# ejcanalesr/multicomponent-T2-toolbox

Hardware: AMD Instinct MI355X
Metric: voxels/sec (whole node) at nTE=32, nT2=60; max |MWF-ref| (higher is better)
Workload: dtype f64

## Files before the change

### multicomponent-t2-toolbox_amd/csrc/fit_kernel.hpp

```cpp
#pragma once
#include <hip/hip_runtime.h>
#include <math.h>
#include <stdint.h>

#include "../../include/met2_hip.h"
#include "abi_common.hpp"
#include "nnls_wave.hpp"
#include "objectives.hpp"

using namespace met2;

struct SortBufs {
    int *key;
    int *perm;
    int *hist;
    int *cursor;
    int *bucket_start;
    int *chunk_start;
    int *queue;
    int *xq;
    int *err;
    int *ovf;
};

#ifndef MET2_BAYES_TABLE
#define MET2_BAYES_TABLE 10
#endif
#define MET2_GCV_LR 6
constexpr int LC_SAVE_DOUBLES = 18;

struct FitArgs {
    int n, m, nfa, kmax, waves, chunk;
    int wave_doubles;
    int method, nlam, maxfun;
    double x2_factor, t2sparc_lambda, xtol;
    double cut_m, cut_ie;
    double lam_lo, lam_hi;
    int all_queued;
    double log_detL;
    const double *Dfa;
    const double *Bfa;
    const double *Dtfa;
    const double *Aq;
    const double *kband;
    const double *lband;
    const double *Kd;
    const double *lam_grid;
    const double *t2s;
    const double *data;
    int64_t vs, es;
    SortBufs sb;
    double *fsol, *sig, *reg, *lam, *maps;
    int32_t *status;
    int64_t nvox;
    const char *seed;
    const double *btab;
    int nbtab, btab_stride;
    double *chol;
    int chol_stride;
    double *big;
    int big_stride;
    double *lc_save;
    int *lc_at;
    int lc_cap;
    double blam[MET2_BAYES_TABLE];
    int test_switches = 0;
    static constexpr int TEST_REFAC_PAIR = 1;
    static constexpr int TEST_SUBST_REF = 2;
    unsigned long long *refac_count = nullptr;
};

#ifndef MET2_UNI_MASK
#define MET2_UNI_MASK 37
#endif
constexpr bool uni_brent(int method, int nb)
{
    const int base = method >= 10 ? method - 10 : method;
    const int bit = base == MET2_X2 ? 0 : ((base == MET2_GCV || base == MET2_GCV_LR) ? 2 : (base == MET2_BAYESREG ? 4 : -1));
    return bit >= 0 && ((MET2_UNI_MASK >> (bit + (nb == 2 ? 1 : 0))) & 1);
}
template <bool PIN>
__device__ __forceinline__ double uni(double v)
{
    if constexpr (PIN) {
    const unsigned long long u = (unsigned long long)__double_as_longlong(v);
    const unsigned lo = (unsigned)__builtin_amdgcn_readfirstlane((int)(unsigned)u), hi = (unsigned)__builtin_amdgcn_readfirstlane((int)(unsigned)(u >> 32));
    return __longlong_as_double((long long)(((unsigned long long)hi << 32) | lo));
    } else return v;
}
#define MET2_UNI_PIN() do { a = uni<PIN>(a); b = uni<PIN>(b); fulc = uni<PIN>(fulc); nfc = uni<PIN>(nfc); xf = uni<PIN>(xf); rat = uni<PIN>(rat); e = uni<PIN>(e); \
                            x = uni<PIN>(x); fx = uni<PIN>(fx); ffulc = uni<PIN>(ffulc); fnfc = uni<PIN>(fnfc); } while (0)

template <bool PIN, class F, class G>
__device__ __forceinline__ double fminbound_dev(F &&fn, G &&on_best, double x1, double x2, double xatol, int maxfun, int &flag)
{
    const double sqrt_eps = sqrt(2.2e-16);
    const double golden_mean = 0.5 * (3.0 - sqrt(5.0));
    double a = x1, b = x2;
    double fulc = a + golden_mean * (b - a);
    double nfc = fulc, xf = fulc;
    double rat = 0.0, e = 0.0;
    double x = xf;
    double fx = fn(x);
    on_best();
    int num = 1;
    flag = 0;
    double fu = INFINITY;
    double ffulc = fx, fnfc = fx;
    double xm = 0.5 * (a + b);
    double tol1 = sqrt_eps * fabs(xf) + xatol / 3.0;
    double tol2 = 2.0 * tol1;
    while (fabs(xf - xm) > (tol2 - 0.5 * (b - a))) {
        bool golden = true;
        if (fabs(e) > tol1) {
            golden = false;
            double r = (xf - nfc) * (fx - ffulc);
            double q = (xf - fulc) * (fx - fnfc);
            double p = (xf - fulc) * q - (xf - nfc) * r;
            q = 2.0 * (q - r);
            if (q > 0.0) p = -p;
            q = fabs(q);
            r = e;
            e = rat;
            if ((fabs(p) < fabs(0.5 * q * r)) && (p > q * (a - xf)) && (p < q * (b - xf))) {
                rat = (p + 0.0) / q;
                x = xf + rat;
                if (((x - a) < tol2) || ((b - x) < tol2)) {
                    double d = xm - xf;
                    double si = (double)((d > 0.0) - (d < 0.0) + (d == 0.0));
                    rat = tol1 * si;
                }
            } else golden = true;
        }
        if (golden) {
            e = (xf >= xm) ? a - xf : b - xf;
            rat = golden_mean * e;
        }
        double si = (double)((rat > 0.0) - (rat < 0.0) + (rat == 0.0));
        double ar = fabs(rat);
        x = xf + si * (ar > tol1 ? ar : tol1);
        MET2_UNI_PIN();
        fu = fn(x);
        num++;
        if (fu <= fx) {
            if (x >= xf) a = xf; else b = xf;
            fulc = nfc; ffulc = fnfc;
            nfc = xf; fnfc = fx;
            xf = x; fx = fu;
            on_best();
        } else {
            if (x < xf) a = x; else b = x;
// ... 547 lines not shown
                    const double ld0 = rec[A.btab_stride - 1];
                    if (fabs(ld0) <= 1.79769313486231570815e308) { tab.U0 = rec; tab.logdet0 = ld0; }
                }
            }
            ++ev;
            return bayes_objective<NB>(S, bd, st, bc, x, b, lane, tab, cholG);
        }, []() {}, BIG ? A.lam_lo : 1e-8, BIG ? A.lam_hi : 2.0, A.xtol, A.maxfun, flag);
        if (flag == 1) stat |= MET2_ST_BRENT_MAXFUN;
        if (bc.failed) stat |= MET2_ST_CHOLFAIL;
        if (!(NB == 2 && (st.itmax_hit & 2))) solve_warm<NB, ONE, BIG>(S, bd, st, lam, true, lane);
        regv = lamv = lam;
    } else if (METHOD == MET2_GCV || METHOD == MET2_GCV_LR) {
        int flag, overflow = 0;
        GcvCache<NB> gc; gc.valid = 0; gc.next = 0;
        if (have_seed) seed_load<NB>(st, A.seed, seed_k, fa, lane);
        double lam = fminbound_dev<uni_brent(METHOD, NB)>([&](double x) {
            if (NB == 2 && (st.itmax_hit & 2)) return 0.0;
            solve_warm<NB, ONE, BIG>(S, bd, st, x, true, lane);
            return gcv_objective<NB, METHOD == MET2_GCV_LR>(S, bd, st, x, b, lane, overflow, gc);
        }, []() {}, BIG ? A.lam_lo : 1e-8, BIG ? A.lam_hi : 10.0, A.xtol, A.maxfun, flag);
        if (flag == 1) stat |= MET2_ST_BRENT_MAXFUN;
        if (overflow) stat |= MET2_ST_KOVERFLOW;
        if (!(NB == 2 && (st.itmax_hit & 2))) solve_warm<NB, ONE, BIG>(S, bd, st, lam, true, lane);
        regv = lamv = lam;
    }
    if (METHOD >= 10) {
        constexpr int BASE = METHOD - 10;
        double SSE = 1.0; BayesCtx bc; bc.failed = 0; bc.log_detL = A.log_detL; bc.beta = 1.0;
        if (BASE == MET2_X2 || BASE == MET2_BAYESREG) {
            nnls_solve<NB>(S, bd, st, 0.0, false, lane);
            SSE = sse_of<NB>(S, st, b, lane);
            int nnz = 0;
#pragma unroll
            for (int bb = 0; bb < NB; ++bb) nnz += __popcll(ballot((lane + 64 * bb < n) && (st.x[bb] > 0.0)));
            double dof = (double)(m - nnz); dof = dof < 1.0 ? 1.0 : dof;
            const double sigma = sqrt(SSE / dof);
            bc.beta = 1.0 / (sigma * sigma);
        }
        double keep = 0.0; int overflow = 0;
        GcvCache<NB> gc; gc.valid = 0; gc.next = 0;
        for (int i = 0; i < A.nlam; ++i) {
            const double x = A.lam_grid[i];
            nnls_solve<NB>(S, bd, st, x, true, lane);
            double val;
            if (BASE == MET2_X2) val = fabs(sse_of<NB>(S, st, b, lane) - A.x2_factor * SSE) / SSE;
            else if (BASE == MET2_GCV || BASE == MET2_GCV_LR) val = gcv_objective<NB, BASE == MET2_GCV_LR>(S, bd, st, x, b, lane, overflow, gc);
            else val = bayes_objective<NB>(S, bd, st, bc, x, b, lane);
            if (lane == i) keep = val;
        }
        if (lane < n) A.fsol[(size_t)v * n + lane] = keep;
        if (NB == 2 && lane + 64 < n) A.fsol[(size_t)v * n + lane + 64] = 0.0;
        if (lane == 0) { A.reg[v] = 0.0; if (A.status) A.status[v] = stat | (overflow ? MET2_ST_KOVERFLOW : 0); }
        return false;
    }
    if (st.itmax_hit & 1) stat |= MET2_ST_ITMAX;
    if (st.itmax_hit & 2) stat |= MET2_ST_KOVERFLOW;
    MET2_CYC_END(0, c_vox);
    MET2_CYC_FLUSH(st);

    double xs[NB];
#pragma unroll
    for (int bb = 0; bb < NB; ++bb) {
        xs[bb] = st.x[bb] * km;
        if (lane + 64 * bb < n) A.fsol[(size_t)v * n + lane + 64 * bb] = xs[bb]; else xs[bb] = 0.0;
    }
    if (A.sig) {
        double sg = model_signal<NB>(S, st, lane) * km;
        if (lane < m) A.sig[(size_t)v * m + lane] = sg;
    }
    if (A.maps) write_metrics<NB>(ml, xs, true, A.maps, A.nvox, v, lane);
    if (lane == 0) {
        A.reg[v] = regv;
        if (A.lam) A.lam[v] = lamv;
        if (A.status) A.status[v] = stat;
    }
    return !BIG && !queued && (st.itmax_hit & 2) != 0;
}

__device__ __forceinline__ void fit_shared(const FitArgs &A, WaveShared &S, double *sR, int wslot)
{
    S.R = sR; S.n = A.n; S.m = A.m; S.kmax = A.kmax; S.rcap = A.wave_doubles; S.K = A.Kd; S.kband = A.kband; S.Dt = nullptr; S.DtG = A.Dtfa; S.dtstride = A.m; S.buffer_rows = true; S.reorder = true; S.have_bdiag = false; S.bdiag[0] = S.bdiag[1] = 0.0;
    S.B = A.Bfa; S.D = A.Dfa; S.bstride = A.n; S.dstride = A.n;
    S.Rg = A.big ? A.big + (size_t)wslot * (size_t)A.big_stride : nullptr; S.gbase = col_base(A.kmax);
    S.refac_pair = (A.test_switches & FitArgs::TEST_REFAC_PAIR) != 0; S.subst_ref = (A.test_switches & FitArgs::TEST_SUBST_REF) != 0; S.refac_count = A.refac_count;
}
template <int METHOD>
__device__ __forceinline__ void fit_shared_fa(const FitArgs &A, WaveShared &S, int fa)
{
    const int n = A.n, m = A.m;
    S.B = A.Bfa + (size_t)fa * n * n; S.D = A.Dfa + (size_t)fa * m * n; S.Dt = A.Dtfa + (size_t)fa * m * n;
    S.DtG = ((METHOD >= 10 ? METHOD - 10 : METHOD) == MET2_GCV_LR) ? A.Aq + (size_t)fa * n * MET2_GCV_LR_RANK : S.Dt;
}

template <int METHOD, int NB>
__device__ __attribute__((noinline)) void fit_voxel_spill(const FitArgs *Ap, big_lds_dp sRl, int64_t v, int fa, int wslot, int qslot, int seed_cap)
{
    const int lane = big_lane();
    double *sR = (double *)sRl;
    FitArgs A;
    {
        static_assert(sizeof(FitArgs) % 4 == 0, "FitArgs is copied word by word");
        const int *src = (const int *)Ap;
        int *dst = (int *)&A;
#pragma unroll
        for (int i = 0; i < (int)(sizeof(FitArgs) / 4); ++i) dst[i] = big_rfl(src[i]);
    }
    v = (int64_t)big_rfl((u64)v); fa = big_rfl(fa); wslot = big_rfl(wslot); qslot = big_rfl(qslot); seed_cap = big_rfl(seed_cap);
    WaveShared S;
    fit_shared(A, S, sR, wslot);
    fit_shared_fa<METHOD>(A, S, fa);
    Band<NB> bd;
    load_band<NB>(bd, A.kband, A.lband, lane);
    MetricLanes<NB> ml;
    metric_lanes<NB>(ml, A.t2s, A.n, A.cut_m, A.cut_ie, lane);
    const int seed_k = (MET2_SEED && A.seed) ? ((const SeedRec *)A.seed)[fa].k : 0;
    const bool have_seed = seed_k > 0 && seed_k <= seed_cap;
    (void)fit_voxel<METHOD, NB, true>(A, S, bd, ml, v, fa, seed_k, have_seed, lane, wslot, qslot);
}

template <int METHOD, int NB, bool SECOND>
__global__ __launch_bounds__(64 * method_max_waves(METHOD, NB)) void fit_kernel(FitArgs A)
{
    extern __shared__ __attribute__((aligned(16))) double smem[];
    const int lane = lane_id(), wave = (int)(threadIdx.x >> 6);
    const int n = A.n, m = A.m, kmax = A.kmax;
    const int tri = A.wave_doubles;
    double *sR = smem + (size_t)wave * tri;

    const int wslot = (int)(blockIdx.x * (unsigned)A.waves + (unsigned)wave);
    WaveShared S;
    fit_shared(A, S, sR, wslot);
    Band<NB> bd;
    load_band<NB>(bd, A.kband, A.lband, lane);
    MetricLanes<NB> ml;
    metric_lanes<NB>(ml, A.t2s, n, A.cut_m, A.cut_ie, lane);

    if constexpr (!SECOND) {
    const int nchunks = A.sb.chunk_start[A.nfa];
    for (int round = 0; round <= nchunks; ++round) {
        int c = nchunks;
        if (lane == 0) {
            const int xcd = (int)(blockIdx.x & 7u);
            for (int t = 0; t < 8; ++t) {
                const int q = (xcd + t) & 7;
                const int qlo = (int)(((int64_t)nchunks * q) >> 3), qhi = (int)(((int64_t)nchunks * (q + 1)) >> 3);
                if (qlo >= qhi) continue;
                const int i = atomicAdd(A.sb.xq + q, 1);
                if (i < qhi - qlo) { c = qlo + i; break; }
            }
        }
        c = __builtin_amdgcn_readfirstlane(c);
        MET2_STAT(5, round);
        if (c >= nchunks) break;
        int lo = 0, hi = A.nfa;
        while (hi - lo > 1) { int mid = (lo + hi) >> 1; if (A.sb.chunk_start[mid] <= c) lo = mid; else hi = mid; }
        const int fa = lo;
        const int first = A.sb.bucket_start[fa] + (c - A.sb.chunk_start[fa]) * A.chunk;
        const int cnt = min(A.chunk, A.sb.bucket_start[fa + 1] - first);
        fit_shared_fa<METHOD>(A, S, fa);
        const int seed_k = (MET2_SEED && A.seed) ? ((const SeedRec *)A.seed)[fa].k : 0;
        const bool have_seed = seed_k > 0 && seed_k <= kmax;
        for (int slot = 0; slot < cnt; ++slot) {
            MET2_STAT(4, slot);
            const int64_t v = A.sb.perm[first + slot];

            if (fit_voxel<METHOD, NB, false>(A, S, bd, ml, v, fa, seed_k, have_seed, lane, wslot, -1) && A.big) {
                if (lane == 0) A.sb.ovf[atomicAdd(A.sb.err + 1, 1)] = (int)v;
// ... 44 lines not shown
```

### multicomponent-t2-toolbox_amd/csrc/met2_fit_nnls_lcurve.hip

```cpp
#ifdef MET2_SPLIT_TU
#define MET2_REFAC_PACKED 1
#include "fit_kernel.hpp"
template int launch_fit_nb<0, 1, false>(const FitArgs &, const LaunchGeom &, hipStream_t);
template int launch_fit_nb<0, 2, false>(const FitArgs &, const LaunchGeom &, hipStream_t);
template int launch_fit_nb<1, 1, false>(const FitArgs &, const LaunchGeom &, hipStream_t);
template int launch_fit_nb<1, 2, false>(const FitArgs &, const LaunchGeom &, hipStream_t);
template int launch_fit_nb<3, 1, false>(const FitArgs &, const LaunchGeom &, hipStream_t);
template int launch_fit_nb<3, 2, false>(const FitArgs &, const LaunchGeom &, hipStream_t);
template int launch_fit_nb<0, 1, true>(const FitArgs &, const LaunchGeom &, hipStream_t);
template int launch_fit_nb<0, 2, true>(const FitArgs &, const LaunchGeom &, hipStream_t);
template int launch_fit_nb<1, 1, true>(const FitArgs &, const LaunchGeom &, hipStream_t);
template int launch_fit_nb<1, 2, true>(const FitArgs &, const LaunchGeom &, hipStream_t);
template int launch_fit_nb<3, 1, true>(const FitArgs &, const LaunchGeom &, hipStream_t);
template int launch_fit_nb<3, 2, true>(const FitArgs &, const LaunchGeom &, hipStream_t);
#endif
```

### multicomponent-t2-toolbox_amd/csrc/met2_fit_x2_nb1.hip

```cpp
#ifdef MET2_SPLIT_TU
#define MET2_REFAC_PACKED 1
#include "fit_kernel.hpp"
template int launch_fit_nb<2, 1, false>(const FitArgs &, const LaunchGeom &, hipStream_t);
template int launch_fit_nb<12, 1, false>(const FitArgs &, const LaunchGeom &, hipStream_t);
#endif
```

### multicomponent-t2-toolbox_amd/csrc/met2_hip.hip

```cpp
#include <hip/hip_runtime.h>
#include <math.h>
#include <stddef.h>
#include <stdint.h>
#include <stdio.h>
#include <stdlib.h>
#include <string.h>
#include <string>
#include <vector>

#include "../../include/met2_hip.h"
#include "abi_common.hpp"
#include "nnls_wave.hpp"
#include "objectives.hpp"
#include "fit_kernel.hpp"

using namespace met2;

#ifdef MET2_SPLIT_TU
extern template int launch_fit_nb<0, 1, false>(const FitArgs &, const LaunchGeom &, hipStream_t);
extern template int launch_fit_nb<0, 2, false>(const FitArgs &, const LaunchGeom &, hipStream_t);
extern template int launch_fit_nb<1, 1, false>(const FitArgs &, const LaunchGeom &, hipStream_t);
extern template int launch_fit_nb<1, 2, false>(const FitArgs &, const LaunchGeom &, hipStream_t);
extern template int launch_fit_nb<2, 1, false>(const FitArgs &, const LaunchGeom &, hipStream_t);
extern template int launch_fit_nb<2, 2, false>(const FitArgs &, const LaunchGeom &, hipStream_t);
// ... 1632 lines not shown
      fprintf(stderr, "[met2] spill-over voxels: solver calls=%llu, with spill-over legs=%llu | cycles plain=%llu spill=%llu (refactor in slot %llu) | appends=%llu removals=%llu refactors=%llu | k start sum=%llu end sum=%llu\n",
              bs[0], bs[1], bs[2], bs[3], bs[9], bs[4], bs[5], bs[6], bs[8], bs[7]); }
#endif
#ifdef MET2_LOOPSTATS
    int ls[8];
    HIPCHK(hipMemcpyFromSymbol(ls, HIP_SYMBOL(met2::g_loopstats), sizeof(ls)));
    fprintf(stderr, "[met2] loop maxima: tries=%d sweeps=%d outer=%d iter=%d taken=%d round=%d jacobi_sweeps=%d last_sweep_rotations=%d\n", ls[0], ls[1], ls[2], ls[3], ls[4], ls[5], ls[6], ls[7]);
#endif
    fflush(stderr);
    return MET2_OK;
}

static int fit_impl(met2_plan *p, int32_t method, int64_t nvox, const double *data, int64_t voxel_stride, int64_t echo_stride,
                    const double *fa_index, const uint8_t *mask, double *fsol, double *sig, double *reg, double *lam, double *maps,
                    int32_t *status, void *stream, bool sync)
{
    if (!p) return fail(MET2_E_INVALID, "NULL plan");
    if (voxel_stride == 0 || echo_stride == 0) return fail(MET2_E_INVALID, "zero stride");
    if (nvox == 0) return MET2_OK;
    if (!data || !fsol || !reg) return fail(MET2_E_INVALID, "NULL argument");
    if (nvox < 0 || nvox > 0x7fffffff) return fail(MET2_E_INVALID, "nvox out of range");
    if (!p->have_dict) return fail(MET2_E_STATE, "no dictionary in the plan");
    if (method != MET2_NNLS && !p->have_pen) return fail(MET2_E_STATE, "no penalty matrix set");
    if (maps && !p->have_t2) return fail(MET2_E_STATE, "metrics requested but no T2 grid set");
    const bool objgrid = method >= 10;
    if (objgrid) { method -= 10; if (method != MET2_X2 && method != MET2_GCV && method != MET2_BAYESREG) return fail(MET2_E_INVALID, "no objective for this method"); }
    if (method < 0 || method > MET2_BAYESREG) return fail(MET2_E_INVALID, "unknown method");
    if (objgrid && p->nlam > p->n_t2) return fail(MET2_E_UNSUPPORTED, "objective grid longer than n_t2");
    USE_DEVICE(p->opt.device);
    hipStream_t s = (hipStream_t)stream;
    if (p->err_pending && p->err_stream != s)
        return fail(MET2_E_STATE, "fits are pending on another stream of this plan: call met2_plan_finish on it first (one plan serves one stream at a time)");
    int rc = ensure_sort_bufs(p, nvox);
    if (rc) return rc;
    const int kmeth = kernel_method(p, method);
    const int kfast = objgrid ? 0 : fast_kmax(p, kmeth);
    LaunchGeom g;
    rc = fit_geometry(p, objgrid ? kmeth + 10 : kmeth, g, kfast, 0, nvox);
    if (rc) return rc;
    if (!p->have_pen) {
        HIPCHK(hipMemsetAsync(p->dKband, 0, sizeof(double) * 5 * 128, s));
        HIPCHK(hipMemsetAsync(p->dLband, 0, sizeof(double) * 5 * 128, s));
        HIPCHK(hipMemsetAsync(p->dKd, 0, sizeof(double) * (size_t)p->n_t2 * p->n_t2, s));
    }
    if (!p->have_t2) HIPCHK(hipMemsetAsync(p->dT2, 0, sizeof(double) * 128, s));
    SortBufs sb = sort_bufs(p);
    hipLaunchKernelGGL(reset_sort_kernel, dim3(1), dim3(256), 0, s, sb, p->n_fa, p->err_pending ? 1 : 0);
    const int nbs = (int)((nvox + MET2_SORT_BLOCK - 1) / MET2_SORT_BLOCK);
    const size_t sort_lds = sizeof(int) * 2 * ((size_t)p->n_fa + 1);
    if (sort_lds > 48 * 1024) {
        if (sort_lds > 150 * 1024) return fail(MET2_E_UNSUPPORTED, "more than 19 000 flip angles (or ROIs) in one plan");
        HIPCHK(hipFuncSetAttribute((const void *)classify_kernel, hipFuncAttributeMaxDynamicSharedMemorySize, (int)sort_lds));
        HIPCHK(hipFuncSetAttribute((const void *)scatter_kernel, hipFuncAttributeMaxDynamicSharedMemorySize, (int)sort_lds));
        HIPCHK(hipFuncSetAttribute((const void *)scan_kernel, hipFuncAttributeMaxDynamicSharedMemorySize, (int)sort_lds));
    }
    int chunk = (method <= MET2_T2SPARC) ? 8 : 1;
    chunk = tuning_env("MET2_CHUNK", 1, 1024, chunk);
    const bool dbg = test_switch("MET2_DEBUG");
    if (dbg) { HIPCHK(hipStreamSynchronize(s)); fprintf(stderr, "[met2] fit: nvox=%lld grid=%d block=%d lds=%d\n", (long long)nvox, g.grid, g.block, g.lds); fflush(stderr); }
    hipLaunchKernelGGL(classify_kernel, dim3(nbs), dim3(MET2_SORT_BLOCK), sort_lds, s, nvox, p->n_te, p->n_fa, data, voxel_stride, echo_stride, fa_index, mask, 1, sb, status);
    hipLaunchKernelGGL(scan_kernel, dim3(1), dim3(256), sort_lds, s, p->n_fa, chunk, sb);
    if (dbg) { HIPCHK(hipStreamSynchronize(s)); fprintf(stderr, "[met2] classify done\n"); fflush(stderr); }
    hipLaunchKernelGGL(scatter_kernel, dim3(nbs), dim3(MET2_SORT_BLOCK), sort_lds, s, nvox, p->n_fa, sb);
    HIPCHK(hipGetLastError());
    if (dbg) {
        HIPCHK(hipStreamSynchronize(s));
        std::vector<int> hs(4 * (size_t)(p->n_fa + 1) + 8);
        HIPCHK(hipMemcpy(hs.data(), p->dSmall, sizeof(int) * hs.size(), hipMemcpyDeviceToHost));
        fprintf(stderr, "[met2] sort done: fitted=%d chunks=%d\n", hs[2 * (p->n_fa + 1) + p->n_fa], hs[3 * (p->n_fa + 1) + p->n_fa]); fflush(stderr);
    }

    FitArgs A;
    A.n = p->n_t2; A.m = p->n_te; A.nfa = p->n_fa; A.kmax = g.kmax; A.waves = g.waves; A.chunk = chunk; A.wave_doubles = g.wave_doubles;
    A.method = method; A.nlam = p->nlam;
    A.maxfun = p->opt.brent_maxfun > 0 ? p->opt.brent_maxfun : (method == MET2_BAYESREG ? 200 : 300);
    A.x2_factor = p->opt.x2_factor; A.t2sparc_lambda = p->opt.t2sparc_lambda; A.xtol = p->opt.brent_xtol;
    A.cut_m = p->opt.t2_myelin_cut; A.cut_ie = p->opt.t2_ie_cut;
    A.lam_lo = method == MET2_GCV ? p->opt.gcv_lo : (method == MET2_BAYESREG ? p->opt.bayes_lo : p->opt.x2_lo);
    A.lam_hi = method == MET2_GCV ? p->opt.gcv_hi : (method == MET2_BAYESREG ? p->opt.bayes_hi : p->opt.x2_hi);
    A.log_detL = p->log_detL;
    A.Dfa = p->dD; A.Bfa = p->dB; A.Dtfa = p->dDt; A.Aq = p->dAq; A.kband = p->dKband; A.lband = p->dLband; A.Kd = p->dKd; A.lam_grid = p->dLam; A.t2s = p->dT2;
    A.data = data; A.vs = voxel_stride; A.es = echo_stride; A.sb = sb; A.fsol = fsol; A.sig = sig; A.reg = reg; A.lam = lam; A.maps = maps; A.status = status; A.nvox = nvox;

    A.test_switches = (test_switch("MET2_REFAC_PAIR") ? FitArgs::TEST_REFAC_PAIR : 0) | (test_switch("MET2_SUBST_REF") ? FitArgs::TEST_SUBST_REF : 0);
    A.refac_count = nullptr;
    if (test_switch("MET2_REFAC_COUNT")) HIPCHK(hipGetSymbolAddress((void **)&A.refac_count, HIP_SYMBOL(g_refac_packed_calls)));
    A.seed = nullptr;
    if (!test_switch("MET2_NO_SEED") && !objgrid && p->have_pen && p->seeds_valid && p->seeds_ok && p->seeds_key[0] == p->opt.t2sparc_lambda &&
        (method == MET2_X2 || method == MET2_GCV || method == MET2_BAYESREG || method == MET2_T2SPARC)) {
        const int slot = method == MET2_BAYESREG ? 1 : (method == MET2_T2SPARC ? 2 : (method == MET2_GCV ? 3 : 0));
        A.seed = p->dSeed + sizeof(SeedRec) * (size_t)slot * p->n_fa;
    }
    A.btab = nullptr; A.nbtab = 0; A.btab_stride = p->btab_stride;
    A.chol = nullptr; A.chol_stride = 0;
    if (method == MET2_BAYESREG && !objgrid && g.nb == 2) {
        const int stride = (col_base(p->n_t2) + 15) & ~15;
        const int64_t need = (int64_t)g.grid * g.waves * stride;
        if (p->cap_chol < need) {
            if (p->dChol) { HIPCHK(hipStreamSynchronize(s)); HIPCHK(hipFree(p->dChol)); p->dChol = nullptr; p->cap_chol = 0; }
            HIPCHK(hipMalloc(&p->dChol, sizeof(double) * (size_t)need));
            p->cap_chol = need;
        }
        A.chol = p->dChol; A.chol_stride = stride;
    }
    A.big = nullptr; A.big_stride = 0;
    if (kfast) {
        const int stride = (col_base(p->n_t2) - col_base(g.kmax) + 15) & ~15;
        LaunchGeom gw;
        rc = fit_geometry(p, kmeth, gw, kfast, 0, -1);
        if (rc) return rc;
        const int64_t need = (int64_t)gw.grid * gw.waves * stride;
        if (p->cap_big < need) {
            if (p->dBig) { HIPCHK(hipStreamSynchronize(s)); HIPCHK(hipFree(p->dBig)); p->dBig = nullptr; p->cap_big = 0; }
            HIPCHK(hipMalloc(&p->dBig, sizeof(double) * (size_t)need));
            p->cap_big = need;
        }
        A.big = p->dBig; A.big_stride = stride;
    }
    A.lc_save = nullptr; A.lc_at = nullptr; A.lc_cap = 0;
    if (A.big && method == MET2_LCURVE && g.nb == 2 && !objgrid && !test_switch("MET2_LC_RESTART")) {
        const int64_t cap = std::min<int64_t>(nvox, std::min<int64_t>(262144, std::max<int64_t>(4096, nvox / 16)));
        const int64_t need = cap * (LC_SAVE_DOUBLES * 64) + (cap + 1) / 2;
        if (p->cap_lc < need) {
            if (p->dLcSave) { HIPCHK(hipStreamSynchronize(s)); HIPCHK(hipFree(p->dLcSave)); p->dLcSave = nullptr; p->cap_lc = 0; }
            HIPCHK(hipMalloc(&p->dLcSave, sizeof(double) * (size_t)need));
            p->cap_lc = need;
        }
        A.lc_save = p->dLcSave; A.lc_at = (int *)(p->dLcSave + cap * (LC_SAVE_DOUBLES * 64)); A.lc_cap = (int)cap;
    }
    for (int j = 0; j < (MET2_BAYES_TABLE > 0 ? MET2_BAYES_TABLE : 1); ++j) A.blam[j] = p->blam[j];
    if (MET2_BAYES_TABLE > 0 && method == MET2_BAYESREG && !objgrid && p->dBtab && p->seeds_valid && p->seeds_ok && !tuning_env("MET2_NO_BAYES_TABLE", 0, 1, 0)) {
        A.btab = p->dBtab; A.nbtab = MET2_BAYES_TABLE;
    }
    const bool custom_iv = !objgrid && ((method == MET2_X2 && (p->opt.x2_lo != 0.0 || p->opt.x2_hi != 10.0)) || (method == MET2_GCV && (p->opt.gcv_lo != 1e-8 || p->opt.gcv_hi != 10.0)) ||
                                        (method == MET2_BAYESREG && (p->opt.bayes_lo != 1e-8 || p->opt.bayes_hi != 2.0)));
    A.all_queued = custom_iv ? 1 : 0;
    HIPCHK(hipEventRecord(p->ev0, s));
    if (objgrid) { A.sig = nullptr; A.maps = nullptr; A.lam = nullptr; }
    if (!custom_iv) {
        rc = launch_method(objgrid ? kmeth + 10 : kmeth, A, g, s);
        if (rc) return rc;
    }
    HIPCHK(hipEventRecord(p->ev1, s));
    const bool spill = A.big || custom_iv;
    if (spill) {
        rc = launch_method(kmeth, A, g, s, true);
        if (rc) return rc;
        HIPCHK(hipEventRecord(p->ev2, s));
    }
    p->timed = true; p->timed2 = spill;
    if (dbg) { rc = debug_counters(method, s); if (rc) return rc; }
    hipLaunchKernelGGL(finalize_unfitted_kernel, dim3(p->cus * 4), dim3(256), 0, s, nvox, p->n_t2, p->n_te, p->dKey, mask, fsol,
                       objgrid ? nullptr : sig, reg, objgrid ? nullptr : lam, objgrid ? nullptr : maps);
    HIPCHK(hipGetLastError());
    HIPCHK(hipMemcpyAsync(p->hErr, sb.err, 4 * sizeof(int), hipMemcpyDeviceToHost, s));
    p->err_pending = true; p->err_stream = s;
    if (!sync) return MET2_OK;
    return met2_plan_finish(p, stream);
}

int met2_fa_bruteforce(met2_plan *p, int64_t nvox, const double *data, const uint8_t *mask, double *fa_index, double *km,
                       double *resid, void *stream)
{
    if (!p) return fail(MET2_E_INVALID, "NULL plan");
    return met2_fa_bruteforce_strided(p, nvox, data, p->n_te, 1, mask, fa_index, km, resid, stream);
}

// ... 220 lines not shown
```

### multicomponent-t2-toolbox_amd/csrc/nnls_wave.hpp

```cpp
#pragma once
#include "wave_ops.hpp"

namespace met2 {

#ifndef MET2_DOUBLE
#define MET2_DOUBLE 0
#endif
#ifndef MET2_REORDER
#define MET2_REORDER 2
#endif

#ifdef MET2_LOOPSTATS
__device__ int g_loopstats[8];
#define MET2_STAT(slot, v) atomicMax(&g_loopstats[slot], (int)(v))
#else
#define MET2_STAT(slot, v)
#endif

#ifdef MET2_CYCSTATS
__device__ unsigned long long g_cyc[16];
__device__ unsigned long long g_ev[40][12];
__device__ unsigned long long g_refk[4];
#define MET2_CYC_BEGIN(var) const unsigned long long var = __builtin_readcyclecounter()
#define MET2_CYC_END(slot, var) st.cyc[slot] += __builtin_readcyclecounter() - var
#define MET2_CYC_ADD(slot, v) st.cyc[slot] += (unsigned long long)(v)
#define MET2_CYC_INIT(st) do { for (int q_ = 0; q_ < 16; ++q_) st.cyc[q_] = 0; } while (0)
#define MET2_CYC_FLUSH(st) do { if (lane_id() == 0) for (int q_ = 0; q_ < 16; ++q_) atomicAdd(&g_cyc[q_], st.cyc[q_]); } while (0)
#else
#define MET2_CYC_BEGIN(var)
#define MET2_CYC_END(slot, var)
#define MET2_CYC_ADD(slot, v)
#define MET2_CYC_INIT(st)
#define MET2_CYC_FLUSH(st)
#endif

struct WaveShared {
    const double *B;
    const double *K;
    const double *Dt;
    const double *DtG;
    const double *kband;
    int dtstride;
    const double *D;
    double *R;
    int n, m, bstride, dstride, kmax;
    int rcap;
    bool have_bdiag;
    double bdiag[2];
    bool reorder;
    bool buffer_rows;
    double *Rg = nullptr;
    int gbase = 0;
    bool refac_pair = false;
    bool subst_ref = false;
    unsigned long long *refac_count = nullptr;
};

template <int NB>
struct Band {
    double lb[NB][5];
};

template <int NB>
struct NnlsState {
    double h[NB];
    double x[NB];
    int pos[NB];
    double y[NB];
    double rinv[NB];
    int ord[NB];
    int k;
    u64 P[NB];
    int itmax_hit;
#ifdef MET2_CYCSTATS
    unsigned long long cyc[16];
#endif
};

__device__ __forceinline__ int row_base(int i, int kmax) { return i * kmax - (i * (i - 1)) / 2 - i; }
__host__ __device__ __forceinline__ constexpr int col_len(int c) { return c + 1; }
__host__ __device__ __forceinline__ constexpr int col_base(int c) { return (c * (c + 1)) >> 1; }

typedef double met2_d2 __attribute__((ext_vector_type(2)));
typedef double met2_d4 __attribute__((ext_vector_type(4)));
typedef const volatile __attribute__((address_space(3))) double *met2_lds_cvp;
__device__ __forceinline__ void lds_quad(const double *p, double &a, double &b, double &c, double &d)
{
    met2_lds_cvp q = (met2_lds_cvp)p;
    a = q[0]; b = q[1]; c = q[2]; d = q[3];
}
__device__ __forceinline__ void lds_pair(const double *p, double &a, double &b)
{
    met2_lds_cvp q = (met2_lds_cvp)p;
    a = q[0]; b = q[1];
}
__device__ __forceinline__ void lds_quad128(const double *p, double &a, double &b, double &c, double &d)
{
    const met2_d2 *q = (const met2_d2 *)__builtin_assume_aligned(p, 16);
    const met2_d2 u = q[0], v = q[1];
    a = u.x; b = u.y; c = v.x; d = v.y;
}

template <int NB>
__device__ __forceinline__ double bcastN(const double (&v)[NB], int idx)
{
    if (NB == 1) return bcast(v[0], idx);
    double t = (idx >> 6) ? v[NB - 1] : v[0];
    return bcast(t, idx & 63);
}
template <int NB>
__device__ __forceinline__ int bcastN_i(const int (&v)[NB], int idx)
{
    if (NB == 1) return bcast_i(v[0], idx);
    int t = (idx >> 6) ? v[NB - 1] : v[0];
    return bcast_i(t, idx & 63);
}
template <int NB>
__device__ __forceinline__ double gatherN(const double (&v)[NB], int src)
{
    double lo = gather(v[0], src & 63);
    if (NB == 1) return lo;
    double hi = gather(v[NB - 1], src & 63);
    return ((src >> 6) & 1) ? hi : lo;
}
template <int NB>
__device__ __forceinline__ int gatherN_i(const int (&v)[NB], int src)
{
    int lo = gather_i(v[0], src & 63);
    if (NB == 1) return lo;
    int hi = gather_i(v[NB - 1], src & 63);
    return ((src >> 6) & 1) ? hi : lo;
}
template <int NB>
__device__ __forceinline__ int first_bit(const u64 (&m)[NB])
{
    if (NB == 1) return first_lane(m[0]);
    return m[0] ? first_lane(m[0]) : 64 + first_lane(m[NB - 1]);
// ... 1085 lines not shown
__device__ __forceinline__ void nnls_solve(const WaveShared &S, const Band<NB> &bd, NnlsState<NB> &st, double lam, bool aug, int lane)
{
    nnls_reset<NB>(st);
    nnls_iterate<NB, ONE, BIG>(S, bd, st, lam, aug ? S.m + S.n : S.m, lane);
}

template <int NB>
__device__ __forceinline__ void reorder_by_x(const WaveShared &S, NnlsState<NB> &st, int lane)
{
    const int k = st.k;
    typedef __attribute__((address_space(3))) unsigned long long *lds_u64p;
    unsigned long long *tabk = (unsigned long long *)S.R;
    int *tabi = (int *)(tabk + k + 4);
    unsigned long long key[NB];
    bool in[NB];
#pragma unroll
    for (int b = 0; b < NB; ++b) {
        const int j = lane + 64 * b;
        in[b] = (st.P[b] >> lane) & 1ull;
        key[b] = ((unsigned long long)__double_as_longlong(st.x[b]) & ~127ull) | (unsigned long long)(127 - j);
        if (in[b]) tabk[st.pos[b]] = key[b];
        if (j >= k && j < k + 4) tabk[j] = 0ull;
    }
    __builtin_amdgcn_wave_barrier();
    int rank[NB];
#pragma unroll
    for (int b = 0; b < NB; ++b) rank[b] = 0;
#pragma clang loop unroll(disable)
    for (int p = 0; p < k; p += 4) {
        const unsigned long long k0 = tabk[p], k1 = tabk[p + 1], k2 = tabk[p + 2], k3 = tabk[p + 3];
#pragma unroll
        for (int b = 0; b < NB; ++b) rank[b] += (int)(k0 > key[b]) + (int)(k1 > key[b]) + (int)(k2 > key[b]) + (int)(k3 > key[b]);
    }
    int zbase = k;
#pragma unroll
    for (int b = 0; b < NB; ++b) {
        const int below = __popcll(~st.P[b] & ((1ull << lane) - 1ull));
        tabi[in[b] ? rank[b] : zbase + below] = lane + 64 * b;
        st.pos[b] = in[b] ? rank[b] : -1;
        zbase += 64 - __popcll(st.P[b]);
    }
    __builtin_amdgcn_wave_barrier();
#pragma unroll
    for (int b = 0; b < NB; ++b) st.ord[b] = min(tabi[lane + 64 * b], S.n - 1);
    __builtin_amdgcn_wave_barrier();
}

template <int NB, int ONE = 0, bool BIG = false>
__device__ __forceinline__ void nnls_solve_warm(const WaveShared &S, const Band<NB> &bd, NnlsState<NB> &st, double lam, bool aug, int lane)
{
    const int kold = st.k;
    if (kold == 0) { nnls_solve<NB, ONE, BIG>(S, bd, st, lam, aug, lane); return; }
    MET2_CYC_BEGIN(c_ref);
    if (NB >= MET2_REORDER && S.reorder && kold >= 4 && S.rcap >= kold + 4 + 32 * NB + 2) reorder_by_x<NB>(S, st, lane);
    if (!refactor<NB, ONE, BIG>(S, bd, st, lam, lane)) {
        MET2_CYC_ADD(4, 1000000000000ull);
        int ordold[NB];
#pragma unroll
        for (int b = 0; b < NB; ++b) { ordold[b] = st.ord[b]; st.pos[b] = -1; st.P[b] = 0ull; }
        st.k = 0;
        for (int p = 0; p < kold; ++p) {
            const int t = bcastN_i<NB>(ordold, p);
            bool okp;
            if constexpr (BIG) okp = (st.k >= S.kmax) ? try_append_big<NB>(S, bd, st, lam, t, lane, true) : try_append<NB>(S, bd, st, lam, t, lane, true);
            else okp = try_append<NB>(S, bd, st, lam, t, lane, true);
            if (!okp) {
#pragma unroll
                for (int b = 0; b < NB; ++b) if (lane + 64 * b == t) st.x[b] = 0.0;
            }
        }
    }
    MET2_CYC_END(1, c_ref);
    MET2_CYC_ADD(12, 1);
    nnls_iterate<NB, ONE, BIG>(S, bd, st, lam, aug ? S.m + S.n : S.m, lane, true);
}

template <int NB>
__device__ __forceinline__ double model_signal(const WaveShared &S, const NnlsState<NB> &st, int lane)
{
    const int k = st.k;
    double acc = 0.0, acc2 = 0.0, xp[NB];
#pragma unroll
    for (int b = 0; b < NB; ++b) { const double t = gatherN<NB>(st.x, st.ord[b]); xp[b] = (lane + 64 * b < k) ? t : 0.0; }
    const unsigned ec = (unsigned)min(lane, S.m - 1);
#pragma clang loop unroll(disable)
    for (int p = 0; p < k; p += 4) {
        double v[4], xs[4];
#pragma unroll
        for (int q = 0; q < 4; ++q) {
            const int pp = p + q;
            v[q] = ld_row_sel(S.buffer_rows, S.Dt, bcastN_i<NB>(st.ord, pp) * S.dtstride, ec);
            xs[q] = bcastN<NB>(xp, pp);
        }
        acc = fma(v[0], xs[0], acc); acc2 = fma(v[1], xs[1], acc2);
        acc = fma(v[2], xs[2], acc); acc2 = fma(v[3], xs[3], acc2);
    }
    return acc + acc2;
}

template <int NB>
__device__ __forceinline__ double sse_of(const WaveShared &S, const NnlsState<NB> &st, double b, int lane)
{
#ifdef MET2_CYCSTATS
    const unsigned long long c0 = __builtin_readcyclecounter();
#endif
    if (MET2_DOUBLE == 3) { const double r0 = model_signal<NB>(S, st, lane); asm volatile("" :: "v"(r0)); }
    double r = model_signal<NB>(S, st, lane) - b;
    r = (lane < S.m) ? r : 0.0;
    const double out = wave_sum(r * r);
#ifdef MET2_CYCSTATS
    const_cast<NnlsState<NB> &>(st).cyc[5] += __builtin_readcyclecounter() - c0;
#endif
    return out;
}

template <int NB>
__device__ __forceinline__ void project(const WaveShared &S, double bvec, int lane, double (&h)[NB]);

template <int NB, bool BIG = false>
__device__ __forceinline__ void refine_csne(const WaveShared &S, NnlsState<NB> &st, double lam, double bvec, int lane)
{
    const int k = st.k;
    if (k == 0) return;
    bool big = false;
    if constexpr (BIG) big = k > S.kmax;
    double r = bvec - model_signal<NB>(S, st, lane);
    r = (lane < S.m) ? r : 0.0;
    double g[NB];
    project<NB>(S, r, lane, g);
    if (lam != 0.0) {
        double kbl[NB][5], kx[NB];
#pragma unroll
        for (int b = 0; b < NB; ++b)
#pragma unroll
            for (int d = 0; d < 5; ++d) kbl[b][d] = S.kband[d * 128 + lane + 64 * b];
        band_mul<NB>(kbl, st.x, lane, kx);
#pragma unroll
        for (int b = 0; b < NB; ++b) g[b] = fma(-lam, kx[b], g[b]);
    }
    double u[NB];
#pragma unroll
    for (int b = 0; b < NB; ++b) { const double t = gatherN<NB>(g, st.ord[b]); u[b] = (lane + 64 * b < k) ? t : 0.0; }
    if (BIG && big) {
        const double *cpl[NB];
#pragma unroll
        for (int b = 0; b < NB; ++b) cpl[b] = big_col(S, min(lane + 64 * b, S.n - 1));
        for (int i = 0; i + 1 < k; ++i) {
            double t[NB];
#pragma unroll
            for (int b = 0; b < NB; ++b) t[b] = u[b] * st.rinv[b];
            const double si = bcastN<NB>(t, i);
#pragma unroll
            for (int b = 0; b < NB; ++b) { const int pl = lane + 64 * b; if (pl > i && pl < k) u[b] = fma(-cpl[b][i], si, u[b]); }
        }
    } else
    for (int i = 0; i + 1 < k; ++i) {
        double t[NB];
#pragma unroll
        for (int b = 0; b < NB; ++b) t[b] = u[b] * st.rinv[b];
        const double si = bcastN<NB>(t, i);
#pragma unroll
        for (int b = 0; b < NB; ++b) { const int pl = lane + 64 * b; if (pl > i && pl < k) u[b] = fma(-S.R[col_base(pl) + i], si, u[b]); }
    }
    double ysave[NB], dl[NB];
#pragma unroll
    for (int b = 0; b < NB; ++b) { ysave[b] = st.y[b]; st.y[b] = (lane + 64 * b < k) ? u[b] * st.rinv[b] : 0.0; }
    if (BIG && big) back_subst_big<NB>(S, st, lane, dl);
    else back_subst<NB>(S, st, lane, dl);
#pragma unroll
    for (int b = 0; b < NB; ++b) st.y[b] = ysave[b];
#pragma unroll
    for (int b = 0; b < NB; ++b) {
        const double d = gatherN<NB>(dl, max(st.pos[b], 0));
        if (st.pos[b] >= 0) st.x[b] += d;
    }
}

__device__ __forceinline__ void big_uniform(WaveShared &S)
{
    S.B = big_rfl(S.B); S.K = big_rfl(S.K); S.Dt = big_rfl(S.Dt); S.DtG = big_rfl(S.DtG); S.kband = big_rfl(S.kband); S.D = big_rfl(S.D);
    S.Rg = big_rfl(S.Rg);
    S.dtstride = big_rfl(S.dtstride); S.n = big_rfl(S.n); S.m = big_rfl(S.m); S.bstride = big_rfl(S.bstride); S.dstride = big_rfl(S.dstride);
    S.kmax = big_rfl(S.kmax); S.rcap = big_rfl(S.rcap); S.gbase = big_rfl(S.gbase);
    S.have_bdiag = big_rfl((int)S.have_bdiag) != 0; S.reorder = big_rfl((int)S.reorder) != 0; S.buffer_rows = big_rfl((int)S.buffer_rows) != 0;
}
template <int NB>
__device__ __forceinline__ void big_uniform(NnlsState<NB> &st)
{
    st.k = big_rfl(st.k); st.itmax_hit = big_rfl(st.itmax_hit);
#pragma unroll
    for (int b = 0; b < NB; ++b) st.P[b] = big_rfl(st.P[b]);
}
template <int NB, int ONE>
__device__ __attribute__((noinline)) void big_solve_fn(WaveShared S, big_lds_dp Rl, Band<NB> bd, NnlsState<NB> *stp, double lam, int flags)
{
    const int lane = big_lane();
    big_uniform(S);
    S.R = (double *)Rl;
    NnlsState<NB> st = *stp;
    big_uniform<NB>(st);
    lam = __hiloint2double(big_rfl(__double2hiint(lam)), big_rfl(__double2loint(lam)));
    flags = big_rfl(flags);
#ifdef MET2_BIGSTATS
    const unsigned long long t0 = __builtin_readcyclecounter();
    const int k0 = st.k;
    st.itmax_hit &= ~4;
#endif
    if (flags & 2) nnls_solve_warm<NB, ONE, true>(S, bd, st, lam, (flags & 1) != 0, lane);
    else nnls_solve<NB, ONE, true>(S, bd, st, lam, (flags & 1) != 0, lane);
#ifdef MET2_BIGSTATS
    {
        const unsigned long long dt = __builtin_readcyclecounter() - t0;
        const bool big = (st.itmax_hit & 4) || k0 > S.kmax;
        MET2_BIGSTAT(0, 1);
        if (big) { MET2_BIGSTAT(1, 1); MET2_BIGSTAT(3, dt); MET2_BIGSTAT(7, st.k); MET2_BIGSTAT(8, k0); } else MET2_BIGSTAT(2, dt);
    }
#endif
    *stp = st;
}
template <int NB>
__device__ __attribute__((noinline)) void big_refine_fn(WaveShared S, big_lds_dp Rl, NnlsState<NB> *stp, double lam, double bvec)
{
    const int lane = big_lane();
    big_uniform(S);
    S.R = (double *)Rl;
    NnlsState<NB> st = *stp;
    big_uniform<NB>(st);
    lam = __hiloint2double(big_rfl(__double2hiint(lam)), big_rfl(__double2loint(lam)));
    refine_csne<NB, true>(S, st, lam, bvec, lane);
    *stp = st;
}

template <int NB>
__device__ __forceinline__ void project(const WaveShared &S, double bvec, int lane, double (&h)[NB])
{
#pragma unroll
    for (int b = 0; b < NB; ++b) h[b] = 0.0;
    unsigned jc[NB];
#pragma unroll
    for (int b = 0; b < NB; ++b) jc[b] = (unsigned)min(lane + 64 * b, S.n - 1);
#pragma clang loop unroll(disable)
    for (int e = 0; e < S.m; e += 4) {
        double dv[4][NB], be[4];
#pragma unroll
        for (int q = 0; q < 4; ++q) {
            const int ee = min(e + q, S.m - 1);
            const double *Drow = S.D + ee * S.dstride;
#pragma unroll
            for (int b = 0; b < NB; ++b) dv[q][b] = Drow[jc[b]];
            be[q] = (e + q < S.m) ? bcast(bvec, ee) : 0.0;
        }
#pragma unroll
        for (int q = 0; q < 4; ++q)
#pragma unroll
            for (int b = 0; b < NB; ++b) h[b] = fma(dv[q][b], be[q], h[b]);
    }
#pragma unroll
    for (int b = 0; b < NB; ++b) h[b] = (lane + 64 * b < S.n) ? h[b] : 0.0;
}

template <int NB, int V>
__device__ __forceinline__ void project_multi(const WaveShared &S, const double (&bvec)[V], int lane, double (&h)[V][NB])
{
    unsigned jc[NB];
#pragma unroll
    for (int b = 0; b < NB; ++b) jc[b] = (unsigned)min(lane + 64 * b, S.n - 1);
#pragma unroll
// ... 39 lines not shown
```

### multicomponent-t2-toolbox_amd/csrc/wave_ops.hpp

```cpp
#pragma once
#include <hip/hip_runtime.h>

namespace met2 {

typedef unsigned long long u64;

__device__ __forceinline__ int lane_id() { return (int)(threadIdx.x & 63u); }

__device__ __forceinline__ int lane_opaque(int lane) { asm volatile("" : "+v"(lane)); return lane; }

__device__ __forceinline__ double bcast(double v, int l)
{
    int lo = __builtin_amdgcn_readlane(__double2loint(v), l);
    int hi = __builtin_amdgcn_readlane(__double2hiint(v), l);
    return __hiloint2double(hi, lo);
}
__device__ __forceinline__ int bcast_i(int v, int l) { return __builtin_amdgcn_readlane(v, l); }

__device__ __forceinline__ double gather(double v, int src)
{
    int lo = __builtin_amdgcn_ds_bpermute(src << 2, __double2loint(v));
    int hi = __builtin_amdgcn_ds_bpermute(src << 2, __double2hiint(v));
    return __hiloint2double(hi, lo);
}
__device__ __forceinline__ int gather_i(int v, int src) { return __builtin_amdgcn_ds_bpermute(src << 2, v); }

template <int CTRL>
__device__ __forceinline__ double dpp_mov(double v)
{
    int lo = __builtin_amdgcn_update_dpp(0, __double2loint(v), CTRL, 0xf, 0xf, true);
    int hi = __builtin_amdgcn_update_dpp(0, __double2hiint(v), CTRL, 0xf, 0xf, true);
    return __hiloint2double(hi, lo);
}

#define MET2_ROW_REDUCE(v, OP)                 \
    v = OP(v, dpp_mov<0xB1>(v));               \
    v = OP(v, dpp_mov<0x4E>(v));               \
    v = OP(v, dpp_mov<0x141>(v));              \
    v = OP(v, dpp_mov<0x140>(v));

__device__ __forceinline__ double op_add(double a, double b) { return a + b; }
__device__ __forceinline__ double op_max(double a, double b) { return fmax(a, b); }
__device__ __forceinline__ double op_min(double a, double b) { return fmin(a, b); }

__device__ __forceinline__ double wave_sum(double v)
{
    MET2_ROW_REDUCE(v, op_add)
    return (bcast(v, 0) + bcast(v, 16)) + (bcast(v, 32) + bcast(v, 48));
}
__device__ __forceinline__ void wave_sum2(double &a, double &b)
{
    MET2_ROW_REDUCE(a, op_add)
    MET2_ROW_REDUCE(b, op_add)
    a = (bcast(a, 0) + bcast(a, 16)) + (bcast(a, 32) + bcast(a, 48));
    b = (bcast(b, 0) + bcast(b, 16)) + (bcast(b, 32) + bcast(b, 48));
}
__device__ __forceinline__ double wave_max(double v)
{
    MET2_ROW_REDUCE(v, op_max)
    return fmax(fmax(bcast(v, 0), bcast(v, 16)), fmax(bcast(v, 32), bcast(v, 48)));
}
__device__ __forceinline__ double wave_min(double v)
{
    MET2_ROW_REDUCE(v, op_min)
    return fmin(fmin(bcast(v, 0), bcast(v, 16)), fmin(bcast(v, 32), bcast(v, 48)));
}

__device__ __forceinline__ u64 ballot(bool p) { return __ballot(p); }
__device__ __forceinline__ int first_lane(u64 m) { return __builtin_ctzll(m); }

}
```

Before: 7.484 million.

## Split the Dt row walk across half-waves and use DPP row broadcasts in reductions

```diff
diff --git a/multicomponent-t2-toolbox_amd/csrc/fit_kernel.hpp b/multicomponent-t2-toolbox_amd/csrc/fit_kernel.hpp
--- a/multicomponent-t2-toolbox_amd/csrc/fit_kernel.hpp
+++ b/multicomponent-t2-toolbox_amd/csrc/fit_kernel.hpp
@@ -67,6 +67,7 @@
     int test_switches = 0;
     static constexpr int TEST_REFAC_PAIR = 1;
     static constexpr int TEST_SUBST_REF = 2;
+    static constexpr int TEST_ROWWALK_REF = 4;
     unsigned long long *refac_count = nullptr;
 };
 
@@ -780,7 +781,8 @@
     S.R = sR; S.n = A.n; S.m = A.m; S.kmax = A.kmax; S.rcap = A.wave_doubles; S.K = A.Kd; S.kband = A.kband; S.Dt = nullptr; S.DtG = A.Dtfa; S.dtstride = A.m; S.buffer_rows = true; S.reorder = true; S.have_bdiag = false; S.bdiag[0] = S.bdiag[1] = 0.0;
     S.B = A.Bfa; S.D = A.Dfa; S.bstride = A.n; S.dstride = A.n;
     S.Rg = A.big ? A.big + (size_t)wslot * (size_t)A.big_stride : nullptr; S.gbase = col_base(A.kmax);
-    S.refac_pair = (A.test_switches & FitArgs::TEST_REFAC_PAIR) != 0; S.subst_ref = (A.test_switches & FitArgs::TEST_SUBST_REF) != 0; S.refac_count = A.refac_count;
+    S.refac_pair = (A.test_switches & FitArgs::TEST_REFAC_PAIR) != 0; S.subst_ref = (A.test_switches & FitArgs::TEST_SUBST_REF) != 0;
+    S.rowwalk_ref = (A.test_switches & FitArgs::TEST_ROWWALK_REF) != 0; S.refac_count = A.refac_count;
 }
 template <int METHOD>
 __device__ __forceinline__ void fit_shared_fa(const FitArgs &A, WaveShared &S, int fa)
diff --git a/multicomponent-t2-toolbox_amd/csrc/met2_fit_nnls_lcurve.hip b/multicomponent-t2-toolbox_amd/csrc/met2_fit_nnls_lcurve.hip
--- a/multicomponent-t2-toolbox_amd/csrc/met2_fit_nnls_lcurve.hip
+++ b/multicomponent-t2-toolbox_amd/csrc/met2_fit_nnls_lcurve.hip
@@ -1,5 +1,6 @@
 #ifdef MET2_SPLIT_TU
 #define MET2_REFAC_PACKED 1
+#define MET2_ROWWALK 1
 #include "fit_kernel.hpp"
 template int launch_fit_nb<0, 1, false>(const FitArgs &, const LaunchGeom &, hipStream_t);
 template int launch_fit_nb<0, 2, false>(const FitArgs &, const LaunchGeom &, hipStream_t);
diff --git a/multicomponent-t2-toolbox_amd/csrc/met2_fit_x2_nb1.hip b/multicomponent-t2-toolbox_amd/csrc/met2_fit_x2_nb1.hip
--- a/multicomponent-t2-toolbox_amd/csrc/met2_fit_x2_nb1.hip
+++ b/multicomponent-t2-toolbox_amd/csrc/met2_fit_x2_nb1.hip
@@ -1,5 +1,6 @@
 #ifdef MET2_SPLIT_TU
 #define MET2_REFAC_PACKED 1
+#define MET2_ROWWALK 1
 #include "fit_kernel.hpp"
 template int launch_fit_nb<2, 1, false>(const FitArgs &, const LaunchGeom &, hipStream_t);
 template int launch_fit_nb<12, 1, false>(const FitArgs &, const LaunchGeom &, hipStream_t);
diff --git a/multicomponent-t2-toolbox_amd/csrc/met2_hip.hip b/multicomponent-t2-toolbox_amd/csrc/met2_hip.hip
--- a/multicomponent-t2-toolbox_amd/csrc/met2_hip.hip
+++ b/multicomponent-t2-toolbox_amd/csrc/met2_hip.hip
@@ -1738,7 +1738,8 @@
     A.Dfa = p->dD; A.Bfa = p->dB; A.Dtfa = p->dDt; A.Aq = p->dAq; A.kband = p->dKband; A.lband = p->dLband; A.Kd = p->dKd; A.lam_grid = p->dLam; A.t2s = p->dT2;
     A.data = data; A.vs = voxel_stride; A.es = echo_stride; A.sb = sb; A.fsol = fsol; A.sig = sig; A.reg = reg; A.lam = lam; A.maps = maps; A.status = status; A.nvox = nvox;
 
-    A.test_switches = (test_switch("MET2_REFAC_PAIR") ? FitArgs::TEST_REFAC_PAIR : 0) | (test_switch("MET2_SUBST_REF") ? FitArgs::TEST_SUBST_REF : 0);
+    A.test_switches = (test_switch("MET2_REFAC_PAIR") ? FitArgs::TEST_REFAC_PAIR : 0) | (test_switch("MET2_SUBST_REF") ? FitArgs::TEST_SUBST_REF : 0) |
+                      (test_switch("MET2_ROWWALK_REF") ? FitArgs::TEST_ROWWALK_REF : 0);
     A.refac_count = nullptr;
     if (test_switch("MET2_REFAC_COUNT")) HIPCHK(hipGetSymbolAddress((void **)&A.refac_count, HIP_SYMBOL(g_refac_packed_calls)));
     A.seed = nullptr;
diff --git a/multicomponent-t2-toolbox_amd/csrc/nnls_wave.hpp b/multicomponent-t2-toolbox_amd/csrc/nnls_wave.hpp
--- a/multicomponent-t2-toolbox_amd/csrc/nnls_wave.hpp
+++ b/multicomponent-t2-toolbox_amd/csrc/nnls_wave.hpp
@@ -53,6 +53,7 @@
     int gbase = 0;
     bool refac_pair = false;
     bool subst_ref = false;
+    bool rowwalk_ref = false;
     unsigned long long *refac_count = nullptr;
 };
 
@@ -1304,6 +1305,20 @@
     double acc = 0.0, acc2 = 0.0, xp[NB];
 #pragma unroll
     for (int b = 0; b < NB; ++b) { const double t = gatherN<NB>(st.x, st.ord[b]); xp[b] = (lane + 64 * b < k) ? t : 0.0; }
+    if constexpr (NB == 1 && MET2_ROWWALK_ON(2)) if (S.m <= 32 && S.buffer_rows && !S.rowwalk_ref) {
+        const int lo_ = lane_opaque(lane), hi = lo_ >> 5;
+        const unsigned ecb = 8u * (unsigned)min(lo_ & 31, S.m - 1), rowb = 8u * (unsigned)S.dtstride;
+#pragma clang loop unroll(disable)
+        for (int p = 0; p < k; p += 4) {
+            const int pa = p + hi, pb = pa + 2;
+            const unsigned ta = (unsigned)gather_i(st.ord[0], pa), tb = (unsigned)gather_i(st.ord[0], pb);
+            const double va = ld_row(S.Dt, 0, ta * rowb + ecb), vb = ld_row(S.Dt, 0, tb * rowb + ecb);
+            const double xa = gather(xp[0], pa), xb = gather(xp[0], pb);
+            acc = fma(va, xa, acc);
+            acc = fma(vb, xb, acc);
+        }
+        return acc + gather(acc, lo_ ^ 32);
+    }
     const unsigned ec = (unsigned)min(lane, S.m - 1);
 #pragma clang loop unroll(disable)
     for (int p = 0; p < k; p += 4) {
@@ -1405,6 +1420,7 @@
     S.dtstride = big_rfl(S.dtstride); S.n = big_rfl(S.n); S.m = big_rfl(S.m); S.bstride = big_rfl(S.bstride); S.dstride = big_rfl(S.dstride);
     S.kmax = big_rfl(S.kmax); S.rcap = big_rfl(S.rcap); S.gbase = big_rfl(S.gbase);
     S.have_bdiag = big_rfl((int)S.have_bdiag) != 0; S.reorder = big_rfl((int)S.reorder) != 0; S.buffer_rows = big_rfl((int)S.buffer_rows) != 0;
+    S.rowwalk_ref = big_rfl((int)S.rowwalk_ref) != 0;
 }
 template <int NB>
 __device__ __forceinline__ void big_uniform(NnlsState<NB> &st)
diff --git a/multicomponent-t2-toolbox_amd/csrc/wave_ops.hpp b/multicomponent-t2-toolbox_amd/csrc/wave_ops.hpp
--- a/multicomponent-t2-toolbox_amd/csrc/wave_ops.hpp
+++ b/multicomponent-t2-toolbox_amd/csrc/wave_ops.hpp
@@ -1,5 +1,16 @@
 #pragma once
 #include <hip/hip_runtime.h>
+
+#if !defined(MET2_ROWWALK) && !defined(MET2_SPLIT_TU)
+#define MET2_ROWWALK 1
+#endif
+#ifndef MET2_ROWWALK
+#define MET2_ROWWALK 0
+#endif
+#ifndef MET2_ROWWALK_PARTS
+#define MET2_ROWWALK_PARTS 6
+#endif
+#define MET2_ROWWALK_ON(bit) (MET2_ROWWALK && (MET2_ROWWALK_PARTS & (bit)))
 
 namespace met2 {
 
@@ -43,27 +54,39 @@
 __device__ __forceinline__ double op_max(double a, double b) { return fmax(a, b); }
 __device__ __forceinline__ double op_min(double a, double b) { return fmin(a, b); }
 
+#if MET2_ROWWALK_ON(4)
+#define MET2_CROSS_ROW(v, OP)                  \
+    v = OP(dpp_mov<0x142>(v), v);              \
+    v = OP(dpp_mov<0x143>(v), v);              \
+    v = bcast(v, 63);
+#else
+#define MET2_CROSS_ROW(v, OP) v = OP(OP(bcast(v, 0), bcast(v, 16)), OP(bcast(v, 32), bcast(v, 48)));
+#endif
+
 __device__ __forceinline__ double wave_sum(double v)
 {
     MET2_ROW_REDUCE(v, op_add)
-    return (bcast(v, 0) + bcast(v, 16)) + (bcast(v, 32) + bcast(v, 48));
+    MET2_CROSS_ROW(v, op_add)
+    return v;
 }
 __device__ __forceinline__ void wave_sum2(double &a, double &b)
 {
     MET2_ROW_REDUCE(a, op_add)
     MET2_ROW_REDUCE(b, op_add)
-    a = (bcast(a, 0) + bcast(a, 16)) + (bcast(a, 32) + bcast(a, 48));
-    b = (bcast(b, 0) + bcast(b, 16)) + (bcast(b, 32) + bcast(b, 48));
+    MET2_CROSS_ROW(a, op_add)
+    MET2_CROSS_ROW(b, op_add)
 }
 __device__ __forceinline__ double wave_max(double v)
 {
     MET2_ROW_REDUCE(v, op_max)
-    return fmax(fmax(bcast(v, 0), bcast(v, 16)), fmax(bcast(v, 32), bcast(v, 48)));
+    MET2_CROSS_ROW(v, op_max)
+    return v;
 }
 __device__ __forceinline__ double wave_min(double v)
 {
     MET2_ROW_REDUCE(v, op_min)
-    return fmin(fmin(bcast(v, 0), bcast(v, 16)), fmin(bcast(v, 32), bcast(v, 48)));
+    MET2_CROSS_ROW(v, op_min)
+    return v;
 }
 
 __device__ __forceinline__ u64 ballot(bool p) { return __ballot(p); }
```

After: 7.692 million, median of 6. 1.03x the previous value.
